# Bioinfo-Tools/PANGEA-plus

Hardware: AMD Instinct MI355X
Metric: classified reads/sec (+ HBM GB/s fraction), 150 bp vs 1 Gbp db, 1/2/4/8 GPU (higher is better)
Workload: dtype u64 (2-bit packed bases, integer scores)

## Files before the change

include/pangea_hip.h:

```cpp
#ifndef PANGEA_HIP_H
#define PANGEA_HIP_H

#include <stddef.h>
#include <stdint.h>

#ifdef __cplusplus
extern "C" {
#endif

typedef enum {
	PGX_OK = 0,
	PGX_E_ARG = -1,
	PGX_E_IO = -2,
	PGX_E_NODEVICE = -3,
	PGX_E_FORMAT = -4,
	PGX_E_NOMEM = -5,
	PGX_E_REFHANG = -6,
	PGX_E_LIMIT = -7
} pgx_status;

const char *pgx_last_error(void);
const char *pgx_version(void);
int pgx_init(int device);
int pgx_device_count(void);
// ... 18 lines not shown
	int64_t n_seq, n_bases;
	int32_t has_amb, index_bits;
	int64_t n_postings;
	int32_t synthetic_ids;
} pgx_db_shape;
int pgx_db_get_shape(const pgx_db *db, pgx_db_shape *out);
int pgx_db_alloc_like(const pgx_db_shape *shape, pgx_db **out);
int pgx_db_finish_import(pgx_db *db);
int pgx_db_checksum(pgx_db *db, uint64_t out[4]);

typedef struct {
	const char *query_path;
	const char *db_prefix;
	const char *out_path;
	int outfmt;
	int rank, world_size;
	int ungapped;
	int no_dust;
} pgx_blastn_opts;
int pgx_blastn_run(const pgx_blastn_opts *opts);
int pgx_db_set_ungapped(pgx_db *db, int ungapped);
int pgx_db_set_dust(pgx_db *db, int dust);
int pgx_db_set_dust_each_search(pgx_db *db, int on);

typedef struct {
	const char *reads_path;
	const char *db_prefix;
	const char *out_path;
	const char *unmapped_path;
	int match_mode;
	int repeat_mode;
	int max_n;
	int report_id;
	const char *reads_b_path;
	const char *unpaired_path;
	int min_insert, max_insert;
} pgx_soap_opts;
int pgx_soap_index(const char *fasta_path);
int pgx_soap_run(const pgx_soap_opts *opts);
int pgx_soap_run_seeded(const pgx_soap_opts *opts, int seed_len, int max_total_mis);

typedef struct pgx_taxdb pgx_taxdb;
typedef struct {
	int32_t tax_id, parent_tax_id;
	int8_t rank;
	char embl_code[3];
// ... 34 lines not shown
	int64_t n_seq;
	int32_t seq_len;
	int64_t n_genus;
	uint64_t read_seed;
	int32_t read_len;
} pgx_synth_cfg;
void pgx_synth_default(pgx_synth_cfg *cfg);
int pgx_db_from_synth(const pgx_synth_cfg *cfg, pgx_db **out);
int pgx_synth_write_taxdump(const pgx_synth_cfg *cfg, const char *dir);

typedef struct pgx_reads pgx_reads;
int pgx_reads_from_fasta(const char *path, int64_t first, int64_t count, pgx_reads **out);
int pgx_reads_from_fasta_text(const char *text, size_t len, int64_t first, int64_t count, pgx_reads **out);
int pgx_reads_from_synth(const pgx_synth_cfg *cfg, int64_t first, int64_t count, pgx_reads **out);
int pgx_reads_write_fasta(const pgx_reads *r, const char *path);
int pgx_reads_redo_dust(pgx_reads *r);
void pgx_reads_close(pgx_reads *r);
int64_t pgx_reads_count(const pgx_reads *r);
int pgx_reads_get(const pgx_reads *r, int64_t i, uint8_t *bases_out, int32_t cap, int32_t *len_out);
int pgx_reads_get_dust(const pgx_reads *r, uint8_t *any_out, uint32_t *woff_out, uint64_t *mask_out, uint64_t *win_f_out,
		       uint64_t *win_r_out, int64_t cap_words, int64_t *n_words_out);
int pgx_db_get_dust(pgx_db *db, const pgx_reads *r, uint8_t *any_out, uint32_t *woff_out, uint64_t *mask_out, uint64_t *win_f_out,
		    uint64_t *win_r_out, int64_t cap_words, int64_t *n_words_out);

typedef struct {
	int32_t read, subject;
	int32_t qstart, qend;
	int32_t sstart, send;
	int32_t score;
	uint16_t mismatch;
	uint16_t gapopen;
} pgx_hit;
#define PGX_HIT_QSPAN(h) ((h).qend - (h).qstart + 1)
#define PGX_HIT_SSPAN(h) (((h).send > (h).sstart ? (h).send - (h).sstart : (h).sstart - (h).send) + 1)
#define PGX_HIT_DIFFS(h) ((PGX_HIT_QSPAN(h) + PGX_HIT_SSPAN(h) - 2 * (h).score - ((PGX_HIT_QSPAN(h) + PGX_HIT_SSPAN(h)) & 1)) / 6)
#define PGX_HIT_GAPS(h) (PGX_HIT_DIFFS(h) - (int32_t)(h).mismatch)
#define PGX_HIT_LENGTH(h) ((PGX_HIT_QSPAN(h) + PGX_HIT_SSPAN(h) + PGX_HIT_GAPS(h)) / 2)

typedef struct pgx_hits pgx_hits;
int pgx_blast_search(pgx_db *db, pgx_reads *reads, pgx_hits **out);
void pgx_hits_close(pgx_hits *h);
int64_t pgx_hits_count(const pgx_hits *h);
int pgx_hits_copy(const pgx_hits *h, pgx_hit *out, int64_t cap);
int pgx_hits_read_offsets(const pgx_hits *h, int64_t *out, int64_t cap);
int pgx_hits_read_counts(const pgx_hits *h, int64_t *out, int64_t cap);
int pgx_hits_slice(const pgx_hits *h, int64_t first_read, int64_t n_reads, pgx_hits **out);
// ... 88 lines not shown
```

pangea-plus_amd/_capi.py:

```python
import ctypes as C
import os
import sys
import threading

import numpy as np

_HERE = os.path.dirname(os.path.abspath(__file__))
lib_path = os.path.join(_HERE, "lib", "libpangea_hip.so")


class PangeaError(RuntimeError):
    def __init__(self, status, msg):
        super().__init__("pangea_hip status %d: %s" % (status, msg))
        self.status = status


_lib = None


def lib():
    global _lib
    if _lib is None:
        if not os.path.exists(lib_path):
            raise PangeaError(-3, "libpangea_hip.so is not built (run `python pangea-plus_amd/build.py`); "
# ... 38 lines not shown
                ("n_postings", C.c_int64), ("synthetic_ids", C.c_int32)]


class _BlastnOpts(C.Structure):
    _fields_ = [("query_path", C.c_char_p), ("db_prefix", C.c_char_p), ("out_path", C.c_char_p), ("outfmt", C.c_int),
                ("rank", C.c_int), ("world_size", C.c_int), ("ungapped", C.c_int), ("no_dust", C.c_int)]


class _SoapOpts(C.Structure):
    _fields_ = [("reads_path", C.c_char_p), ("db_prefix", C.c_char_p), ("out_path", C.c_char_p),
                ("unmapped_path", C.c_char_p), ("match_mode", C.c_int), ("repeat_mode", C.c_int), ("max_n", C.c_int),
                ("report_id", C.c_int), ("reads_b_path", C.c_char_p), ("unpaired_path", C.c_char_p), ("min_insert", C.c_int),
                ("max_insert", C.c_int)]


HIT_DTYPE = np.dtype([("read", "<i4"), ("subject", "<i4"), ("qstart", "<i4"), ("qend", "<i4"), ("sstart", "<i4"),
                      ("send", "<i4"), ("score", "<i4"), ("mismatch", "<u2"), ("gapopen", "<u2")])
REC_DTYPE = np.dtype([("hit", "<i4"), ("matches", "<i4")])
VOTE_DTYPE = np.dtype([("depth", "<i4"), ("name", "<u4", (7,)), ("votes", "u1", (7,)), ("pad", "u1")])

SYMBOLS = [
    "pgx_last_error", "pgx_version", "pgx_init", "pgx_device_count", "pgx_current_device", "pgx_db_build", "pgx_db_open",
    "pgx_db_from_fasta", "pgx_db_close", "pgx_db_num_seqs", "pgx_db_num_bases", "pgx_db_seq_id",
    "pgx_db_device_arrays", "pgx_db_get_shape", "pgx_db_alloc_like", "pgx_db_finish_import", "pgx_db_checksum", "pgx_blastn_run", "pgx_db_set_ungapped", "pgx_db_set_dust", "pgx_db_set_dust_each_search",
    "pgx_soap_index", "pgx_soap_run", "pgx_soap_run_seeded", "pgx_tax_create", "pgx_tax_open", "pgx_tax_close", "pgx_tax_gi2taxid",
    "pgx_tax_node", "pgx_tax_names", "pgx_tax_format_node", "pgx_tax_format_name", "pgx_tax_cli", "pgx_free",
    "pgx_tax_lineage_batch", "pgx_taxcollect_file", "pgx_consensus_file", "pgx_synth_default", "pgx_db_from_synth",
    "pgx_synth_write_taxdump", "pgx_reads_from_fasta", "pgx_reads_from_fasta_text", "pgx_reads_from_synth", "pgx_reads_write_fasta", "pgx_reads_redo_dust", "pgx_rdp_write_file", "pgx_reads_close", "pgx_reads_count",
    "pgx_reads_get", "pgx_reads_get_dust", "pgx_db_get_dust", "pgx_blast_search", "pgx_hits_close", "pgx_hits_count", "pgx_hits_copy",
    "pgx_hits_read_offsets", "pgx_hits_read_counts", "pgx_hits_slice", "pgx_hits_format", "pgx_db_bind_taxonomy", "pgx_db_subject_lineage",
    "pgx_rdp_from_file", "pgx_rdp_from_synth", "pgx_rdp_close", "pgx_consensus_batch", "pgx_classify_consensus", "pgx_classify_consensus_tri", "pgx_vote3_batch", "pgx_vote3_format",
    "pgx_consensus_format", "pgx_consensus_format_file", "pgx_last_stage_times", "pgx_megaclust_file", "pgx_megaclust_batch", "pgx_megaclustable", "pgx_unclas_file", "pgx_unclassified_batch", "pgx_trim_file", "pgx_trim_reads", "pgx_blast_score_columns", "pgx_blast_score_columns_v", "pgx_probe_gather", "pgx_probe_issue", "pgx_probe_issue_name",
]


def _declare(L):
    def sig(name, restype=C.c_int, argtypes=None):
        f = getattr(L, name, None)
        if f is None:
            return
        f.restype = restype
        if argtypes is not None:
            f.argtypes = argtypes
    V, I64, I32, S = C.c_void_p, C.c_int64, C.c_int32, C.c_char_p
    sig("pgx_last_error", S)
    sig("pgx_version", S)
    sig("pgx_db_num_seqs", I64, [V])
    sig("pgx_db_num_bases", I64, [V])
    sig("pgx_db_seq_id", S, [V, I64])
    sig("pgx_db_subject_lineage", S, [V, I64])
    sig("pgx_db_set_ungapped", C.c_int, [V, C.c_int])
    sig("pgx_db_set_dust_each_search", C.c_int, [V, C.c_int])
    sig("pgx_reads_count", I64, [V])
    sig("pgx_hits_count", I64, [V])
    sig("pgx_reads_from_synth", C.c_int, [V, I64, I64, V])
    sig("pgx_reads_from_fasta", C.c_int, [S, I64, I64, V])
    sig("pgx_reads_from_fasta_text", C.c_int, [C.c_char_p, C.c_size_t, I64, I64, V])
    sig("pgx_reads_get", C.c_int, [V, I64, V, I32, V])
    sig("pgx_reads_get_dust", C.c_int, [V, V, V, V, V, V, I64, V])
    sig("pgx_db_get_dust", C.c_int, [V, V, V, V, V, V, V, I64, V])
    sig("pgx_reads_write_fasta", C.c_int, [V, S])
    sig("pgx_reads_redo_dust", C.c_int, [V])
    sig("pgx_rdp_write_file", C.c_int, [V, V, V, S])
    sig("pgx_hits_copy", C.c_int, [V, V, I64])
    sig("pgx_hits_read_offsets", C.c_int, [V, V, I64])
    sig("pgx_hits_read_counts", C.c_int, [V, V, I64])
    sig("pgx_rdp_from_synth", C.c_int, [V, I64, I64, V, V])
    sig("pgx_consensus_batch", C.c_int, [V, V, V, V, I64])
    sig("pgx_classify_consensus", C.c_int, [V, V, V, V, V, I64])
    sig("pgx_classify_consensus_tri", C.c_int, [V, V, V, C.c_char_p, V, V, I64])
    sig("pgx_vote3_batch", C.c_int, [V, V, V, V, C.c_char_p, V, I64])
    sig("pgx_vote3_format", C.c_int, [V, V, V, I64, V, V])
    sig("pgx_consensus_format", C.c_int, [V, V, V, V, I64, V, V])
    sig("pgx_consensus_format_file", C.c_int, [V, V, V, V, I64, S, V])
    sig("pgx_tax_lineage_batch", C.c_int, [V, V, I64, V, V, V])
# ... 123 lines not shown
        s = _DbShape()
        _check(lib().pgx_db_get_shape(self.ptr, C.byref(s)))
        return (s.n_seq, s.n_bases, s.has_amb, s.index_bits, s.n_postings, s.synthetic_ids)

    def checksum(self):
        out = (C.c_uint64 * 4)()
        _check(lib().pgx_db_checksum(self.ptr, out))
        return tuple(int(x) for x in out)

    def device_arrays(self):
        arr = (_DevArray * 16)()
        n = _check(lib().pgx_db_device_arrays(self.ptr, arr, 16))
        return [(arr[i].name.decode(), _CudaArray(arr[i].ptr, arr[i].bytes, self)) for i in range(n)]

    def set_ungapped(self, flag=True):
        _check(lib().pgx_db_set_ungapped(self.ptr, 1 if flag else 0))

    def set_dust(self, flag=True):
        _check(lib().pgx_db_set_dust(self.ptr, 1 if flag else 0))

    def set_dust_each_search(self, flag):
        _check(lib().pgx_db_set_dust_each_search(self.ptr, 1 if flag else 0))

    def dust_bits(self, reads):
        return _dust_bits(lambda *a: lib().pgx_db_get_dust(self.ptr, reads.ptr, *a), len(reads))

    def bind_taxonomy(self, tax):
        _check(lib().pgx_db_bind_taxonomy(self.ptr, tax.ptr))

    def subject_lineage(self, i):
        s = lib().pgx_db_subject_lineage(self.ptr, i)
        return None if s is None else s.decode("latin-1")


def _dust_bits(call, n):
    n_words = C.c_int64()
    _check(call(None, None, None, None, None, 0, C.byref(n_words)))
    nw = n_words.value
    any_ = np.zeros(n, dtype=np.uint8)
    woff = np.zeros(n + 1, dtype=np.uint32)
    mask, win_f, win_r = (np.zeros(max(nw, 1), dtype=np.uint64) for _ in range(3))
    _check(call(any_.ctypes.data, woff.ctypes.data, mask.ctypes.data, win_f.ctypes.data, win_r.ctypes.data, nw, None))
    return any_, woff, mask[:nw], win_f[:nw], win_r[:nw]


class Reads(_Handle):
# ... 342 lines not shown
```

pangea-plus_amd/csrc/classify.hip:

```cpp
#include <algorithm>
#include <chrono>

#include "bitops.hpp"
#include "consensus_core.hpp"
#include "engine.hpp"

namespace pgx {

struct Diag {
	const uint64_t *rw, *ra;
	const uint64_t *dbw, *dba;
	int64_t dstart;
	int lo, hi;
};

template <bool AMB> __device__ __forceinline__ uint64_t mmw(const Diag &D, int w)
{
	int b0 = 32 * w;
	if (b0 + 32 <= D.lo || b0 >= D.hi)
		return kEven;
	uint64_t x = D.rw[w] ^ window64(D.dbw, D.dstart + b0);
	uint64_t m = (x | (x >> 1)) & kEven;
	if (AMB) {
		if (D.ra)
			m |= D.ra[w];
		if (D.dba)
			m |= window64(D.dba, D.dstart + b0);
	}
// ... 229 lines not shown
				return lo - 1;
			w--;
			m = mmw<AMB>(D, w);
		}
		int r = 32 * w + ((63 - __clzll((long long)m)) >> 1);
		return r >= lo ? r : lo - 1;
	}
	struct Fwd {
		int k;
	};
	__device__ __forceinline__ Fwd fwd_from(int k) const { return Fwd{ k }; }
	__device__ __forceinline__ int fwd_next(Fwd &c) const { return c.k = first_ge(c.k + 1); }
	struct Bwd {
		int k;
	};
	__device__ __forceinline__ Bwd bwd_from(int k) const { return Bwd{ k }; }
	__device__ __forceinline__ int bwd_next(Bwd &c) const { return c.k = last_lt(c.k); }
};

constexpr int kStage = 128;
constexpr int kDeal = 2;
constexpr int kQueue = 64 * (kDeal + 1);
constexpr int kWavesPerBlock = 4;

typedef uint32_t u32x4 __attribute__((ext_vector_type(4)));
union HitWords {
	pgx_hit h;
	u32x4 v[2];
};
__device__ __forceinline__ void store_hit_stream(pgx_hit *p, const pgx_hit &h)
{
	HitWords w;
	w.h = h;
	u32x4 *d = reinterpret_cast<u32x4 *>(p);
	__builtin_nontemporal_store(w.v[0], d);
	__builtin_nontemporal_store(w.v[1], d + 1);
}


constexpr int kDiagSlots = 128;
constexpr int kDiagProbes = 8;
constexpr uint32_t kNoDiag = 0xFFFFFFFFu;

struct WaveLds {
	union {
		pgx_hit hit[kStage];
// ... 280 lines not shown
					}
				}
				h.qstart = (int32_t)woff;
				h.qend = anchor;
				h.sstart = (int32_t)(uint32_t)(D.dstart + anchor);
				h.send = strand | (b0l << 1) | (b0r << 12);
				h.score = L;
				h.mismatch = (uint16_t)kl;
				h.gapopen = (uint16_t)kr;
			}
			if (PGX_DBG_STOP(db) != 7)
				emit(h);
			covered = br + 1;
		}
		if constexpr (Mask::kHasWindows) {
			pos = Mask::win_first_ge(W, covered > e ? covered : e + 1);
			if (uw && pos < D.hi)
				pos = M.last_lt(pos) + 1;
		} else
			pos = covered > e + 1 ? covered : e + 1;
	}
}

__device__ __forceinline__ void lds_fence()
{
	asm volatile("s_waitcnt lgkmcnt(0)" ::: "memory");
	__builtin_amdgcn_wave_barrier();
}

template <bool AMB, int NW, bool LISTED, bool DUST>
__global__ __launch_bounds__(64 * kWavesPerBlock, NW == 8 ? 3 : 4) void k_seed_extend(DbView db, ReadsView rd, OutView ov,
								      uint32_t *__restrict__ read_cnt,
								      uint32_t *__restrict__ read_start)
{
	constexpr bool DENSE = NW > 0;
	constexpr int RPW = DENSE ? 2 : 1;
	constexpr int LPR = 64 / RPW;
	constexpr unsigned int SLOT_CAP = kStage;
	__shared__ WaveLds s_lds[kWavesPerBlock];
	const int wave = threadIdx.x >> 6, lane = threadIdx.x & 63;
	const int my_rs = lane / LPR, my_li = lane % LPR;
	WaveLds *st = &s_lds[wave];
	unsigned long long n_probe = 0, n_post = 0, n_runs = 0, n_main = 0, n_surv = 0;
	unsigned long long chunk_base = 0;
	unsigned int chunk_used = kChunk;
	const unsigned long long lt_mask = lane ? (~0ull >> (64 - lane)) : 0ull;

	for (uint32_t rbase = (blockIdx.x * kWavesPerBlock + wave) * RPW; rbase < rd.n; rbase += gridDim.x * kWavesPerBlock * RPW) {
		const bool hasB = RPW == 2 && rbase + 1 < rd.n;
		const uint32_t rA = LISTED ? rd.list[rbase] : rbase, rB = LISTED ? (hasB ? rd.list[rbase + 1] : 0u) : rbase + 1;
		const int LA = (int)rd.len[rA], LB = hasB ? (int)rd.len[rB] : 0;
		const uint32_t wA = rd.woff[rA], wB = hasB ? rd.woff[rB] : 0u;
		const int L = my_rs ? LB : LA;
		const uint32_t w0 = my_rs ? wB : wA;
		const int nps = L >= kSeedK ? (L - kSeedK) / kProbeStride + 1 : 0;
		const int P = 2 * nps;
		const int PA = LA >= kSeedK ? 2 * ((LA - kSeedK) / kProbeStride + 1) : 0;
		const int PB = LB >= kSeedK ? 2 * ((LB - kSeedK) / kProbeStride + 1) : 0;
		const int Pmax = PA > PB ? PA : PB;
		unsigned int emitted[2] = { 0, 0 }, q_n = 0;
		bool frag[2] = { false, false };
		if (lane == 0) {
			st->n[0] = st->n[1] = 0;
			st->direct[0] = st->direct[1] = 0;
		}
		if (RPW == 2) {
#pragma unroll
			for (int k = 0; k < 2 * kDiagSlots / 64; k++)
				(&st->diag[0][0][0])[k * 64 + lane] = kNoDiag;
		}
		const bool dustA = DUST && rd.dustwin_f && rd.dust_any[rA] != 0, dustB = DUST && rd.dustwin_f && hasB && rd.dust_any[rB] != 0;
// ... 959 lines not shown
	v.n_bases = db->n_bases;
	v.bits = db->index_bits;
	v.gapped = db->ungapped ? 0 : 1;
	v.deep_from = kGapDeepFrom;
#ifdef PGX_STAGE_PROBES
	v.dbg_stop = getenv("PGX_SEED_STOP") ? atoi(getenv("PGX_SEED_STOP")) : 0;
#else
	v.dbg_stop = 0;
#endif
	return v;
}

static ReadsView reads_view(const pgx_reads *rd)
{
	ReadsView v;
	v.fwd = rd->d_fwd.data();
	v.rc = rd->d_rc.data();
	v.fwd_amb = rd->has_amb ? rd->d_fwd_amb.data() : nullptr;
	v.rc_amb = rd->has_amb ? rd->d_rc_amb.data() : nullptr;
	v.len = rd->d_len.data();
	v.woff = rd->d_woff.data();
	v.n = (uint32_t)rd->n;
	v.list = nullptr;
	v.dustwin_f = rd->has_dust ? rd->dustb.win_f.data() : nullptr;
	v.dustwin_r = rd->has_dust ? rd->dustb.win_r.data() : nullptr;
	v.dust_any = rd->has_dust ? rd->dustb.any.data() : nullptr;
	return v;
}

static ConsView cons_view(const pgx_db *db, const pgx_rdp *rdp)
{
	ConsView cv;
	memset(&cv, 0, sizeof cv);
#ifdef PGX_STAGE_PROBES
	cv.dbg = getenv("PGX_SORT_STOP") ? atoi(getenv("PGX_SORT_STOP")) : 0;
#else
	cv.dbg = 0;
#endif
	if (db && db->bound) {
		cv.subj_tok_off = db->d_subj_tok_off.data();
		cv.subj_tok = db->d_subj_tok.data();
		cv.tok_rank = db->d_tok_rank.data();
		cv.subj_pairs = db->d_subj_pairs.data();
		cv.pair_words = db->pair_words;
		cv.simrank_lut = db->d_simrank_lut.data();
		cv.simrank_len = db->d_simrank_len.data();
		cv.simrank_undef = db->simrank_undef;
		cv.simrank_zero = db->simrank_zero;
	}
	cv.np_max = db ? db->max_pairs : 15;
	cv.nr_max = rdp ? rdp->max_trip : kRdpRegs;
	if (rdp) {
		cv.rdp_off = rdp->d_off.data();
		cv.rdp_name = rdp->d_name.data();
		cv.rdp_rank = rdp->d_rank.data();
		cv.rdp_present = rdp->d_present.data();
		cv.rdp_code = rdp->d_code.data();
	}
	return cv;
}

struct StageEvents {
	static constexpr int kN = 8;
	hipEvent_t e[kN] = {};
	bool ok = false;
	int init()
	{
		if (ok)
			return 0;
		for (auto &x : e)
			PGX_HIP(hipEventCreate(&x));
		ok = true;
		return 0;
	}
	void mark(int i, hipStream_t s) { (void)hipEventRecord(e[i], s); }
	float ms(int a, int b) const
	{
		float t = 0;
		(void)hipEventElapsedTime(&t, e[a], e[b]);
		return t;
	}
};

__global__ __launch_bounds__(256) void k_merge_pieces(const pgx_hit *__restrict__ scratch, const uint32_t *__restrict__ piece_start,
						      const uint32_t *__restrict__ piece_off, const uint32_t *__restrict__ parent,
						      const uint32_t *__restrict__ qoff, uint32_t n_pieces, pgx_hit *__restrict__ hits,
// ... 26 lines not shown
	if (r > n_reads)
		return;
	const uint32_t o = piece_off[piece_first[r]];
	read_off[r] = o;
	if (r < n_reads) {
		read_cnt[r] = piece_off[piece_first[r + 1]] - o;
		read_start[r] = kFragmented;
	}
}

struct Workspace {
	hipStream_t stream = nullptr;
	StageEvents ev;
	DevBuf<unsigned long long> counters;
	unsigned long long *h_counters = nullptr;
	DevBuf<pgx_hit> scratch, ovf;
	DevBuf<uint8_t> scratch_key, ovf_key;
	DevBuf<uint8_t> scratch_reg;
	DevBuf<uint32_t> partial, cursor, big_list, read_start, mid_list;
	DevBuf<uint32_t> piece_cnt, piece_off, parent_start;
	DevBuf<pgx_consensus_rec> recs;
	GappedWork gapped;
	DustBufs dust;
	pgx_hits hits;
	uint64_t hit_cap_hint = 0, ovf_cap_hint = 0;
	double table_per_read_hint = 0.0;
	pgx_stage_times times;
	int device = -1;
	~Workspace()
	{
		if (h_counters)
			(void)hipHostFree(h_counters);
		if (stream)
			(void)hipStreamDestroy(stream);
	}
};
constexpr int kNCounters = 12;

static int workspace_of(pgx_db *db, Workspace **out)
{
	if (!db->work) {
		auto w = std::make_shared<Workspace>();
		PGX_HIP(hipGetDevice(&w->device));
		PGX_HIP(hipStreamCreate(&w->stream));
		PGX_HIP(hipHostMalloc((void **)&w->h_counters, (kNCounters + 3) * sizeof(unsigned long long)));
		PGX_TRY(w->ev.init());
		PGX_TRY(w->counters.alloc(kNCounters, 0, 0, true));
		db->work = w;
	}
	*out = static_cast<Workspace *>(db->work.get());
	return 0;
}

int db_stream(pgx_db *db, hipStream_t *out)
{
	Workspace *ws = nullptr;
	PGX_TRY(workspace_of(db, &ws));
	*out = ws->stream;
	return 0;
}

int search_pipeline(pgx_db *db, pgx_reads *rd, const pgx_rdp *rdp, pgx_hits *out, pgx_consensus_rec *d_recs)
{
	PGX_TRY(require_device());
	if (rdp && !db->bound)
		return fail(PGX_E_ARG, "consensus needs pgx_db_bind_taxonomy() first");
	if (rdp && rdp->n != rd->n)
		return fail(PGX_E_ARG, "RDP stream holds %lld reads, batch holds %lld", (long long)rdp->n, (long long)rd->n);
	std::lock_guard<std::mutex> lock(db->search_mu);
	static const bool laps_on = getenv("PGX_CALL_LAPS") != nullptr;
	const auto lap_t0 = std::chrono::steady_clock::now();
	auto lap = [&](const char *what) {
		if (laps_on)
			fprintf(stderr, "[pgx lap] %8.2f ms  %s\n", std::chrono::duration<double, std::milli>(std::chrono::steady_clock::now() - lap_t0).count(), what);
	};
	trace_point("search_pipeline: entered");
	Workspace *wsp = nullptr;
	PGX_TRY(workspace_of(db, &wsp));
	Workspace &ws = *wsp;
	hipStream_t st = ws.stream;
	pgx_stage_times &tm = ws.times;
	memset(&tm, 0, sizeof tm);
	const uint64_t n = (uint64_t)rd->n;
	out->n_reads = rd->n;
	PGX_TRY(out->d_read_cnt.ensure(n + 1));
	PGX_TRY(out->d_read_off.ensure(n + 1));
	if (n == 0) {
		out->n_hits = 0;
		t_times = tm;
		return 0;
	}
	index_check(db, "search_pipeline");
	const DbView dv = db_view(db);
	const bool split = rd->pieces && rd->pieces->n > 0;
	const pgx_reads *sr = split ? rd->pieces.get() : rd;
	const uint64_t ns = (uint64_t)sr->n;
	if (split) {
		PGX_TRY(ws.piece_cnt.ensure(ns + 1));
		PGX_TRY(ws.piece_off.ensure(ns + 1));
		PGX_TRY(ws.parent_start.ensure(n));
	}
	ReadsView rv = reads_view(sr);
	if (!db->dust)
		rv.dustwin_f = rv.dustwin_r = nullptr;
	const int grid = (int)std::min<uint64_t>((n + kWavesPerBlock - 1) / kWavesPerBlock, 256ull * 8);
// ... 9 lines not shown
	bool long_reads = false;
	for (auto &c : classes)
		long_reads = long_reads || c.words == 0;
	const uint32_t n_part = (uint32_t)((ns + kScanBlock * kScanItems - 1) / (kScanBlock * kScanItems));
	PGX_TRY(ws.partial.ensure(n_part));
	PGX_TRY(ws.cursor.ensure(ns));
	PGX_TRY(ws.big_list.ensure(n));
	PGX_TRY(ws.mid_list.ensure(n + 64ull * kWavesPerBlock * 256 * 8));
	trace_point("search_pipeline: lists ready");
	const ConsView cv = cons_view(db, rdp);
	const int lds_ok = rd->max_len <= 65535 ? 1 : 0;
	uint64_t H = 0, H_ovf = 0;
	ws.ev.mark(6, st);
	const bool dust_now = db->dust && db->dust_each_search;
	if (dust_now) {
		PGX_TRY(reads_dust_again(sr, ws.dust, st));
		if (sr->has_dust) {
			rv.dustwin_f = ws.dust.win_f.data();
			rv.dustwin_r = ws.dust.win_r.data();
			rv.dust_any = ws.dust.any.data();
		}
	}
	ws.ev.mark(7, st);
	for (int attempt = 0;; attempt++) {
		if (attempt > 8)
			return fail(PGX_E_LIMIT, "hit tables did not settle after %d attempts", attempt);
		PGX_TRY(scratch.ensure(cap));
		PGX_TRY(ovf.ensure(ovf_cap));
		trace_point("search_pipeline: seed tables ready");
		PGX_TRY(out->d_hits.ensure(table_cap));
		trace_point("search_pipeline: hit table ready");
		cap = scratch.n;
		ovf_cap = ovf.n;
		if (dv.gapped) {
			PGX_TRY(ws.scratch_key.ensure(cap + 16));
			PGX_TRY(ws.scratch_reg.ensure(cap + 16));
			PGX_TRY(ws.ovf_key.ensure(ovf_cap));
			PGX_HIP(hipMemsetAsync(ws.scratch_key.data(), 0xFF, cap + 16, st));
		}
		table_cap = out->d_hits.n;
		PGX_HIP(hipMemsetAsync(ws.counters.data(), 0, kNCounters * sizeof(unsigned long long), st));
		OutView ov;
		ov.main = scratch.data();
		ov.ovf = ovf.data();
		ov.main_key = ws.scratch_key.data();
		ov.ovf_key = ws.ovf_key.data();
		ov.main_reg = ws.scratch_reg.data();
		ov.reg_shift = gapped_region_shift(db->n_bases);
		ov.main_cap = cap;
		ov.ovf_cap = ovf_cap;
		ov.counters = ws.counters.data();
		uint32_t *big_count = reinterpret_cast<uint32_t *>(ws.counters.data() + 8), *mid_count = reinterpret_cast<uint32_t *>(ws.counters.data() + 9);
		trace_point("search_pipeline: tables ready");
		lap("tables ready");
		ws.ev.mark(0, st);
		uint32_t *rc_ptr = split ? ws.piece_cnt.data() : out->d_read_cnt.data(), *rs_ptr = read_start.data();
		for (const pgx_reads::SearchClass &c0 : classes) {
			pgx_reads::SearchClass c = c0;
			c.amb = c.amb || db->has_amb;
			ReadsView cvw = rv;
			const uint64_t cn = c.count;
			cvw.n = (uint32_t)cn;
			cvw.list = c.listed ? sr->d_class_list.data() + c.off : nullptr;
			const int per_block = kWavesPerBlock * (c.words > 0 ? 2 : 1);
			const dim3 g((unsigned)std::min<uint64_t>((cn + per_block - 1) / per_block, 256ull * 8)), b(64 * kWavesPerBlock);
#define PGX_SEED_LAUNCH2(A, W, D)                                                                                                  \
	do {                                                                                                                       \
		if (c.listed)                                                                                                      \
			hipLaunchKernelGGL((k_seed_extend<A, W, true, D>), g, b, 0, st, dv, cvw, ov, rc_ptr, rs_ptr);             \
		else                                                                                                               \
			hipLaunchKernelGGL((k_seed_extend<A, W, false, D>), g, b, 0, st, dv, cvw, ov, rc_ptr, rs_ptr);            \
	} while (0)
#define PGX_SEED_LAUNCH(A, W)                                                                                                      \
	do {                                                                                                                       \
		if (c.dust && cvw.dustwin_f)                                                                                       \
			PGX_SEED_LAUNCH2(A, W, true);                                                                              \
		else                                                                                                               \
			PGX_SEED_LAUNCH2(A, W, false);                                                                             \
	} while (0)
			if (c.amb && c.words == 3)
				PGX_SEED_LAUNCH(true, 3);
			else if (c.amb && c.words == 5)
				PGX_SEED_LAUNCH(true, 5);
			else if (c.amb && c.words == 8)
				PGX_SEED_LAUNCH(true, 8);
			else if (c.amb)
// ... 86 lines not shown
			again = true;
			tm.grown |= 4;
		}
		if (!again && H > table_cap) {
			table_cap = H + H / 16;
			again = true;
			tm.grown |= 8;
		}
		tm.attempts = attempt + 1;
		if (!again)
			break;
	}
	ws.hit_cap_hint = std::max<uint64_t>(ws.hit_cap_hint, h_cnt[0] + h_cnt[0] / 16);
	ws.ovf_cap_hint = std::max<uint64_t>(ws.ovf_cap_hint, H_ovf + H_ovf / 16);
	ws.table_per_read_hint = std::max(ws.table_per_read_hint, (double)(H + H / 16) / (double)std::max(n, ns));
	out->n_hits = (int64_t)H;
	out->gapped = dv.gapped != 0;
	tm.hits = (int64_t)H;
	tm.probes = (int64_t)h_cnt[1];
	tm.postings = (int64_t)h_cnt[2];
	tm.candidates = (int64_t)h_cnt[3];
	tm.survivors = (int64_t)h_cnt[6];
	tm.gapped_wide = (int64_t)(uint32_t)h_cnt[kNCounters] + (int64_t)(uint32_t)(h_cnt[kNCounters + 2] >> 32);
	tm.seed_extend_ms = ws.ev.ms(0, 1);
	tm.gapped_ms = ws.ev.ms(1, 2);
	tm.group_ms = ws.ev.ms(2, 3);
	tm.sort_ms = ws.ev.ms(3, 4);
	tm.total_ms = ws.ev.ms(0, 4);
	tm.dust_ms = dust_now ? ws.ev.ms(6, 7) : 0.0f;
	tm.total_ms += tm.dust_ms;
	const unsigned long long hit_limit = getenv("PGX_HIT_LIMIT") ? strtoull(getenv("PGX_HIT_LIMIT"), nullptr, 10) : (1ull << 32);
	if (H >= hit_limit)
		return fail(PGX_E_LIMIT, "%llu hits in one batch exceed the 32-bit slot limit: use smaller batches",
			    (unsigned long long)H);
	const uint32_t n_big = (uint32_t)h_cnt[8];
	if (n_big) {
		const uint32_t *sort_start = split ? ws.parent_start.data() : read_start.data();
		ws.ev.mark(4, st);
		PGX_TRY(sort_big_reads(out->d_hits.data(), scratch.data(), sort_start, out->d_read_off.data(), out->d_read_cnt.data(),
				       ws.big_list.data(), n_big, dv.gapped != 0));
		if (rdp) {
			hipLaunchKernelGGL(k_consensus_serial, dim3((n_big + 63) / 64), dim3(64), 0, 0, out->d_hits.data(), out->d_read_off.data(),
					   out->d_read_cnt.data(), ws.big_list.data(), n_big, cv, d_recs);
			PGX_HIP(hipGetLastError());
		}
		ws.ev.mark(5, 0);
		PGX_HIP(hipDeviceSynchronize());
		const float extra = ws.ev.ms(4, 5);
		tm.sort_ms += extra;
		tm.total_ms += extra;
	}
// ... 71 lines not shown
	}
	return pgx_classify_consensus(db, reads, rdp, hits_out, out, cap);
}

int pgx_db_get_dust(pgx_db *db, const pgx_reads *r, uint8_t *any_out, uint32_t *woff_out, uint64_t *mask_out, uint64_t *win_f_out,
		    uint64_t *win_r_out, int64_t cap_words, int64_t *n_words_out)
{
	if (!db || !r)
		return fail(PGX_E_ARG, "pgx_db_get_dust: null argument");
	if (r->pieces && r->pieces->n > 0)
		return fail(PGX_E_ARG, "pgx_db_get_dust: the batch is searched piece by piece, the handle's bits describe the pieces");
	std::lock_guard<std::mutex> lock(db->search_mu);
	if (!db->work)
		return fail(PGX_E_ARG, "pgx_db_get_dust: no search has run through this handle");
	const Workspace &ws = *static_cast<const Workspace *>(db->work.get());
	return dust_read_back("pgx_db_get_dust", r, ws.dust, ws.stream, any_out, woff_out, mask_out, win_f_out, win_r_out, cap_words, n_words_out);
}

int pgx_db_set_dust_each_search(pgx_db *db, int on)
{
	if (!db)
		return fail(PGX_E_ARG, "pgx_db_set_dust_each_search: null argument");
	db->dust_each_search = on != 0;
	return 0;
}

int pgx_db_set_ungapped(pgx_db *db, int ungapped)
{
	if (!db)
		return fail(PGX_E_ARG, "pgx_db_set_ungapped: null argument");
	std::lock_guard<std::mutex> lock(db->search_mu);
	db->ungapped = ungapped != 0;
	return 0;
}

int pgx_db_set_dust(pgx_db *db, int dust)
{
	if (!db)
		return fail(PGX_E_ARG, "pgx_db_set_dust: null argument");
	std::lock_guard<std::mutex> lock(db->search_mu);
	db->dust = dust != 0;
	return 0;
}

void pgx_hits_close(pgx_hits *h) { delete h; }
int64_t pgx_hits_count(const pgx_hits *h) { return h ? h->n_hits : 0; }
// ... 69 lines not shown
```

pangea-plus_amd/csrc/engine.hpp:

```cpp
#pragma once
#include <memory>
#include <functional>
#include <thread>
#include <atomic>
#include <mutex>
#include <string>
#include <unordered_map>
#include <vector>

#include "common.hpp"
#include "rdp_host.hpp"

struct pgx_db {
	int64_t n_seq = 0, n_bases = 0;
	bool has_amb = false;
	bool synthetic_ids = false;
	std::vector<uint32_t> h_seq_off;
	std::vector<std::string> ids;
	std::vector<uint64_t> h_words, h_amb;

	pgx::DevBuf<uint64_t> d_words, d_amb;
	pgx::DevBuf<uint32_t> d_seq_off, d_blk_subj;
	pgx::DevBuf<uint4> d_blk_info;
	pgx::DevBuf<uint32_t> d_amb_blk;
	int index_bits = 0;
	int64_t n_postings = 0;
	std::shared_ptr<void> work;
	std::mutex search_mu;
	bool dust = true;
	bool dust_each_search = false;
	bool ungapped = false;
	pgx::DevBuf<uint32_t> d_bucket_off, d_postings;
	pgx::DevBuf<uint3> d_post_ctx;

	bool bound = false;
	std::vector<std::string> lineage;
	std::vector<std::string> token_text;
	std::unordered_map<std::string, uint32_t> token_id;
	pgx::DevBuf<uint32_t> d_subj_tok_off, d_subj_tok;
	pgx::DevBuf<int8_t> d_tok_rank;
	pgx::DevBuf<uint32_t> d_subj_pairs;
	int max_pairs = 15;
	int pair_words = 16;
	std::vector<int8_t> h_tok_rank;
	std::vector<int32_t> subj_taxid;
	std::vector<std::string> lin_text;
	pgx::DevBuf<uint32_t> d_subj_lin;
	uint32_t empty_lin = 0;
	pgx::DevBuf<uint32_t> d_node_name_tok;
	pgx::DevBuf<uint32_t> d_simrank_lut;
	pgx::DevBuf<uint32_t> d_simrank_len;
	uint32_t simrank_undef = 0, simrank_zero = 0;
	uint32_t intern(const std::string &s);
// ... 165 lines not shown
#endif

struct DbView {
	const uint64_t *words, *amb;
	const uint32_t *seq_off, *blk_subj, *bucket_off, *postings;
	const uint4 *blk_info;
	const uint3 *post_ctx;
	const uint32_t *amb_blk;
	uint32_t n_seq;
	int64_t n_bases;
	int bits;
	int gapped;
	int deep_from;
	int dbg_stop;
};

struct ReadsView {
	const uint64_t *fwd, *rc, *fwd_amb, *rc_amb;
	const uint64_t *dustwin_f, *dustwin_r;
	const uint8_t *dust_any;
	const uint32_t *len, *woff;
	uint32_t n;
	const uint32_t *list;
};


constexpr uint32_t kFragmented = 0xFFFFFFFFu;

struct GappedWork {
	DevBuf<unsigned long long> big_list, big_list2;
	DevBuf<uint32_t> big_count;
	DevBuf<uint2> side_list;
	DevBuf<uint32_t> order;
	DevBuf<uint32_t> items, bins;
	DevBuf<uint32_t> items1;
	DevBuf<uint8_t> keys1;
};
int gapped_stage(const DbView &dv, const ReadsView &rv, pgx_hit *main_table, const uint8_t *main_key, const uint32_t *read_start,
		 const uint32_t *read_cnt, pgx_hit *ovf_table, const uint8_t *ovf_key, const unsigned long long *ovf_count, unsigned long long ovf_cap, bool long_reads,
		 unsigned long long hit_cap, int max_len, GappedWork &gw, hipStream_t stream, const unsigned long long *main_used, const uint8_t *main_reg);
constexpr int kGapDeepFrom = 320;
inline int gapped_region_shift(int64_t n_bases)
{
	int s = 0;
	while (((n_bases + 1024) >> s) > 240)
		s++;
// ... 22 lines not shown
```

Baseline: 136.0 million.

## Sort reads by probable database locus before seeding and hand them out by ticket

Adds a pre-pass that looks up one or two 16-mers of each read in the seed index, takes the first posting's database position as a coarse bin, and radix-sorts reads by that bin. The seed/extend kernel then walks the sorted list, pulling work from an atomic ticket counter instead of a static stride. The aim is that waves running at the same time touch nearby database regions, which should improve cache reuse of the reference words and posting lists, and that dynamic ticketing should balance load. This costs an extra key kernel, a rocprim sort, some buffers and an atomic per grab. It only switches on automatically for large batches against large databases.

```diff
diff --git a/include/pangea_hip.h b/include/pangea_hip.h
--- a/include/pangea_hip.h
+++ b/include/pangea_hip.h
@@ -64,6 +64,7 @@
 int pgx_db_set_ungapped(pgx_db *db, int ungapped);
 int pgx_db_set_dust(pgx_db *db, int dust);
 int pgx_db_set_dust_each_search(pgx_db *db, int on);
+int pgx_db_set_read_order(pgx_db *db, int mode);
 
 typedef struct {
 	const char *reads_path;
@@ -144,6 +145,7 @@
 		       uint64_t *win_r_out, int64_t cap_words, int64_t *n_words_out);
 int pgx_db_get_dust(pgx_db *db, const pgx_reads *r, uint8_t *any_out, uint32_t *woff_out, uint64_t *mask_out, uint64_t *win_f_out,
 		    uint64_t *win_r_out, int64_t cap_words, int64_t *n_words_out);
+int pgx_db_get_read_order(pgx_db *db, const pgx_reads *r, uint32_t *order_out, uint32_t *key_out, int64_t cap, int64_t *n_out);
 
 typedef struct {
 	int32_t read, subject;
diff --git a/pangea-plus_amd/_capi.py b/pangea-plus_amd/_capi.py
--- a/pangea-plus_amd/_capi.py
+++ b/pangea-plus_amd/_capi.py
@@ -84,7 +84,7 @@
 SYMBOLS = [
     "pgx_last_error", "pgx_version", "pgx_init", "pgx_device_count", "pgx_current_device", "pgx_db_build", "pgx_db_open",
     "pgx_db_from_fasta", "pgx_db_close", "pgx_db_num_seqs", "pgx_db_num_bases", "pgx_db_seq_id",
-    "pgx_db_device_arrays", "pgx_db_get_shape", "pgx_db_alloc_like", "pgx_db_finish_import", "pgx_db_checksum", "pgx_blastn_run", "pgx_db_set_ungapped", "pgx_db_set_dust", "pgx_db_set_dust_each_search",
+    "pgx_db_device_arrays", "pgx_db_get_shape", "pgx_db_alloc_like", "pgx_db_finish_import", "pgx_db_checksum", "pgx_blastn_run", "pgx_db_set_ungapped", "pgx_db_set_dust", "pgx_db_set_dust_each_search", "pgx_db_set_read_order", "pgx_db_get_read_order",
     "pgx_soap_index", "pgx_soap_run", "pgx_soap_run_seeded", "pgx_tax_create", "pgx_tax_open", "pgx_tax_close", "pgx_tax_gi2taxid",
     "pgx_tax_node", "pgx_tax_names", "pgx_tax_format_node", "pgx_tax_format_name", "pgx_tax_cli", "pgx_free",
     "pgx_tax_lineage_batch", "pgx_taxcollect_file", "pgx_consensus_file", "pgx_synth_default", "pgx_db_from_synth",
@@ -113,6 +113,8 @@
     sig("pgx_db_subject_lineage", S, [V, I64])
     sig("pgx_db_set_ungapped", C.c_int, [V, C.c_int])
     sig("pgx_db_set_dust_each_search", C.c_int, [V, C.c_int])
+    sig("pgx_db_set_read_order", C.c_int, [V, C.c_int])
+    sig("pgx_db_get_read_order", C.c_int, [V, V, V, V, I64, V])
     sig("pgx_reads_count", I64, [V])
     sig("pgx_hits_count", I64, [V])
     sig("pgx_reads_from_synth", C.c_int, [V, I64, I64, V])
@@ -282,6 +284,17 @@
     def set_dust_each_search(self, flag):
         _check(lib().pgx_db_set_dust_each_search(self.ptr, 1 if flag else 0))
 
+    def set_read_order(self, mode):
+        _check(lib().pgx_db_set_read_order(self.ptr, int(mode)))
+
+    def read_order(self, reads):
+        n = C.c_int64()
+        _check(lib().pgx_db_get_read_order(self.ptr, reads.ptr, None, None, 0, C.byref(n)))
+        order, keys = np.zeros(n.value, dtype=np.uint32), np.zeros(n.value, dtype=np.uint32)
+        if n.value:
+            _check(lib().pgx_db_get_read_order(self.ptr, reads.ptr, order.ctypes.data, keys.ctypes.data, n.value, C.byref(n)))
+        return order, keys
+
     def dust_bits(self, reads):
         return _dust_bits(lambda *a: lib().pgx_db_get_dust(self.ptr, reads.ptr, *a), len(reads))
 
diff --git a/pangea-plus_amd/csrc/classify.hip b/pangea-plus_amd/csrc/classify.hip
--- a/pangea-plus_amd/csrc/classify.hip
+++ b/pangea-plus_amd/csrc/classify.hip
@@ -4,6 +4,9 @@
 #include "bitops.hpp"
 #include "consensus_core.hpp"
 #include "engine.hpp"
+#include "read_order.hpp"
+
+#include <rocprim/device/device_radix_sort.hpp>
 
 namespace pgx {
 
@@ -279,6 +282,7 @@
 constexpr int kDeal = 2;
 constexpr int kQueue = 64 * (kDeal + 1);
 constexpr int kWavesPerBlock = 4;
+constexpr int kOrderGrab = 4;
 
 typedef uint32_t u32x4 __attribute__((ext_vector_type(4)));
 union HitWords {
@@ -605,6 +609,49 @@
 	}
 }
 
+struct OrderIndexView {
+	const uint32_t *bucket_off, *postings;
+	int bits;
+	__device__ __forceinline__ OrderRange range(uint32_t kmer) const
+	{
+		const uint32_t b = seed_bucket(kmer, bits);
+		const uint32_t lo = __builtin_nontemporal_load(&bucket_off[b]);
+		return OrderRange{ lo, __builtin_nontemporal_load(&bucket_off[(uint64_t)b + 1]) - lo };
+	}
+	__device__ __forceinline__ uint32_t first(uint32_t lo) const { return __builtin_nontemporal_load(&postings[lo]); }
+};
+
+__global__ __launch_bounds__(256) void k_read_order_keys(DbView db, ReadsView rd, int shift, uint32_t last_bin, uint32_t cls,
+							 uint32_t *__restrict__ keys, uint32_t *__restrict__ vals)
+{
+	const uint32_t i = blockIdx.x * blockDim.x + threadIdx.x;
+	if (i >= rd.n)
+		return;
+	const uint32_t r = rd.list ? rd.list[i] : i;
+	const int L = (int)rd.len[r];
+	uint32_t kmer[2][2] = { { 0, 0 }, { 0, 0 } };
+	bool usable[2][2] = { { false, false }, { false, false } };
+	if (L >= kOrderProbeLen) {
+		const uint32_t w0 = rd.woff[r];
+		const bool two = L >= kOrderProbe1 + kOrderProbeLen;
+#pragma unroll
+		for (int s = 0; s < 2; s++) {
+			const uint64_t *rw = (s ? rd.rc : rd.fwd) + w0;
+			const uint64_t *ra = s ? rd.rc_amb : rd.fwd_amb;
+			const uint64_t a = ra ? ra[w0] : 0ull;
+			kmer[s][0] = window16(rw, kOrderProbe0);
+			usable[s][0] = (uint32_t)a == 0u;
+			if (two) {
+				kmer[s][1] = window16(rw, kOrderProbe1);
+				usable[s][1] = (uint32_t)(a >> (2 * kOrderProbe1)) == 0u;
+			}
+		}
+	}
+	const OrderIndexView ix = { db.bucket_off, db.postings, db.bits };
+	keys[i] = read_order_key(ix, kmer, usable, shift, last_bin) | (cls << 16);
+	vals[i] = r;
+}
+
 __device__ __forceinline__ void lds_fence()
 {
 	asm volatile("s_waitcnt lgkmcnt(0)" ::: "memory");
@@ -629,7 +676,22 @@
 	unsigned int chunk_used = kChunk;
 	const unsigned long long lt_mask = lane ? (~0ull >> (64 - lane)) : 0ull;
 
-	for (uint32_t rbase = (blockIdx.x * kWavesPerBlock + wave) * RPW; rbase < rd.n; rbase += gridDim.x * kWavesPerBlock * RPW) {
+	uint32_t t_next = 0, t_end = 0;
+	auto next_round = [&](uint32_t cur) -> uint32_t {
+		if (!LISTED || !rd.ticket)
+			return cur + gridDim.x * kWavesPerBlock * RPW;
+		if (t_next == t_end) {
+			uint32_t t = 0;
+			if (lane == 0)
+				t = atomicAdd(rd.ticket, (uint32_t)(kOrderGrab * RPW));
+			t_next = __builtin_amdgcn_readfirstlane(t);
+			t_end = t_next + kOrderGrab * RPW;
+		}
+		const uint32_t r = t_next;
+		t_next += RPW;
+		return r;
+	};
+	for (uint32_t rbase = LISTED && rd.ticket ? next_round(0) : (blockIdx.x * kWavesPerBlock + wave) * RPW; rbase < rd.n; rbase = next_round(rbase)) {
 		const bool hasB = RPW == 2 && rbase + 1 < rd.n;
 		const uint32_t rA = LISTED ? rd.list[rbase] : rbase, rB = LISTED ? (hasB ? rd.list[rbase + 1] : 0u) : rbase + 1;
 		const int LA = (int)rd.len[rA], LB = hasB ? (int)rd.len[rB] : 0;
@@ -1635,6 +1697,7 @@
 	v.woff = rd->d_woff.data();
 	v.n = (uint32_t)rd->n;
 	v.list = nullptr;
+	v.ticket = nullptr;
 	v.dustwin_f = rd->has_dust ? rd->dustb.win_f.data() : nullptr;
 	v.dustwin_r = rd->has_dust ? rd->dustb.win_r.data() : nullptr;
 	v.dust_any = rd->has_dust ? rd->dustb.any.data() : nullptr;
@@ -1674,7 +1737,7 @@
 }
 
 struct StageEvents {
-	static constexpr int kN = 8;
+	static constexpr int kN = 10;
 	hipEvent_t e[kN] = {};
 	bool ok = false;
 	int init()
@@ -1747,6 +1810,10 @@
 	DevBuf<pgx_consensus_rec> recs;
 	GappedWork gapped;
 	DustBufs dust;
+	DevBuf<uint32_t> order_key_in, order_val_in, order_key, order_list;
+	DevBuf<uint8_t> order_tmp;
+	DevBuf<uint32_t> order_ticket;
+	uint64_t order_n = 0;
 	pgx_hits hits;
 	uint64_t hit_cap_hint = 0, ovf_cap_hint = 0;
 	double table_per_read_hint = 0.0;
@@ -1782,6 +1849,63 @@
 	Workspace *ws = nullptr;
 	PGX_TRY(workspace_of(db, &ws));
 	*out = ws->stream;
+	return 0;
+}
+
+constexpr uint64_t kOrderMinReads = 1u << 22;
+constexpr uint64_t kOrderMinDbBytes = 32ull << 20;
+static bool order_wanted(const pgx_db *db, uint64_t class_reads)
+{
+	if (db->read_order == 1)
+		return class_reads > 0;
+	if (db->read_order == 2)
+		return false;
+	return class_reads >= kOrderMinReads && (uint64_t)db->n_bases / 4 >= kOrderMinDbBytes;
+}
+
+static int order_reads(const pgx_db *db, const DbView &dv, const ReadsView &rv, const pgx_reads *sr, Workspace &ws,
+		       std::vector<int64_t> &ordered)
+{
+	hipStream_t st = ws.stream;
+	const std::vector<pgx_reads::SearchClass> &classes = sr->classes;
+	ordered.assign(classes.size(), -1);
+	const int shift = read_order_shift(dv.n_bases), key_bits = read_order_key_bits(dv.n_bases);
+	const uint32_t last_bin = read_order_last_bin(dv.n_bases);
+	uint64_t total = 0;
+	size_t tmp_bytes = 0;
+	for (size_t c = 0; c < classes.size(); c++)
+		if (order_wanted(db, classes[c].count)) {
+			ordered[c] = (int64_t)total;
+			total += classes[c].count;
+			size_t bytes = 0;
+			PGX_HIP(rocprim::radix_sort_pairs(nullptr, bytes, (uint32_t *)nullptr, (uint32_t *)nullptr, (uint32_t *)nullptr, (uint32_t *)nullptr,
+							  (size_t)classes[c].count, 0, key_bits, st));
+			tmp_bytes = std::max(tmp_bytes, bytes);
+		}
+	ws.order_n = total;
+	if (total == 0)
+		return 0;
+	PGX_TRY(ws.order_key_in.ensure(total));
+	PGX_TRY(ws.order_val_in.ensure(total));
+	PGX_TRY(ws.order_key.ensure(total));
+	PGX_TRY(ws.order_list.ensure(total));
+	PGX_TRY(ws.order_tmp.ensure(tmp_bytes ? tmp_bytes : 1));
+	PGX_TRY(ws.order_ticket.ensure(classes.size()));
+	for (size_t c = 0; c < classes.size(); c++) {
+		if (ordered[c] < 0)
+			continue;
+		const uint64_t o = (uint64_t)ordered[c], cn = classes[c].count;
+		ReadsView cvw = rv;
+		cvw.n = (uint32_t)cn;
+		cvw.list = classes[c].listed ? sr->d_class_list.data() + classes[c].off : nullptr;
+		hipLaunchKernelGGL(k_read_order_keys, dim3((unsigned)((cn + 255) / 256)), dim3(256), 0, st, dv, cvw, shift, last_bin, (uint32_t)c,
+				   ws.order_key_in.data() + o, ws.order_val_in.data() + o);
+		PGX_HIP(hipGetLastError());
+		size_t bytes = ws.order_tmp.n;
+		PGX_HIP(rocprim::radix_sort_pairs(ws.order_tmp.data(), bytes, ws.order_key_in.data() + o, ws.order_key.data() + o,
+						  ws.order_val_in.data() + o, ws.order_list.data() + o, (size_t)cn, 0, key_bits, st));
+	}
+	trace_point("order_reads");
 	return 0;
 }
 
@@ -1806,6 +1930,7 @@
 	hipStream_t st = ws.stream;
 	pgx_stage_times &tm = ws.times;
 	memset(&tm, 0, sizeof tm);
+	ws.order_n = 0;
 	const uint64_t n = (uint64_t)rd->n;
 	out->n_reads = rd->n;
 	PGX_TRY(out->d_read_cnt.ensure(n + 1));
@@ -1861,6 +1986,11 @@
 		}
 	}
 	ws.ev.mark(7, st);
+	std::vector<int64_t> ordered;
+	PGX_TRY(order_reads(db, dv, rv, sr, ws, ordered));
+	const bool order_now = ws.order_n > 0;
+	if (order_now)
+		ws.ev.mark(8, st);
 	for (int attempt = 0;; attempt++) {
 		if (attempt > 8)
 			return fail(PGX_E_LIMIT, "hit tables did not settle after %d attempts", attempt);
@@ -1892,15 +2022,22 @@
 		uint32_t *big_count = reinterpret_cast<uint32_t *>(ws.counters.data() + 8), *mid_count = reinterpret_cast<uint32_t *>(ws.counters.data() + 9);
 		trace_point("search_pipeline: tables ready");
 		lap("tables ready");
+		if (order_now)
+			PGX_HIP(hipMemsetAsync(ws.order_ticket.data(), 0, classes.size() * sizeof(uint32_t), st));
 		ws.ev.mark(0, st);
 		uint32_t *rc_ptr = split ? ws.piece_cnt.data() : out->d_read_cnt.data(), *rs_ptr = read_start.data();
-		for (const pgx_reads::SearchClass &c0 : classes) {
-			pgx_reads::SearchClass c = c0;
+		for (size_t ci = 0; ci < classes.size(); ci++) {
+			pgx_reads::SearchClass c = classes[ci];
 			c.amb = c.amb || db->has_amb;
 			ReadsView cvw = rv;
 			const uint64_t cn = c.count;
 			cvw.n = (uint32_t)cn;
 			cvw.list = c.listed ? sr->d_class_list.data() + c.off : nullptr;
+			if (ordered[ci] >= 0) {
+				c.listed = true;
+				cvw.list = ws.order_list.data() + ordered[ci];
+				cvw.ticket = ws.order_ticket.data() + ci;
+			}
 			const int per_block = kWavesPerBlock * (c.words > 0 ? 2 : 1);
 			const dim3 g((unsigned)std::min<uint64_t>((cn + per_block - 1) / per_block, 256ull * 8)), b(64 * kWavesPerBlock);
 #define PGX_SEED_LAUNCH2(A, W, D)                                                                                                  \
@@ -2033,11 +2170,11 @@
 	tm.candidates = (int64_t)h_cnt[3];
 	tm.survivors = (int64_t)h_cnt[6];
 	tm.gapped_wide = (int64_t)(uint32_t)h_cnt[kNCounters] + (int64_t)(uint32_t)(h_cnt[kNCounters + 2] >> 32);
-	tm.seed_extend_ms = ws.ev.ms(0, 1);
+	tm.seed_extend_ms = ws.ev.ms(0, 1) + (order_now ? ws.ev.ms(7, 8) : 0.0f);
 	tm.gapped_ms = ws.ev.ms(1, 2);
 	tm.group_ms = ws.ev.ms(2, 3);
 	tm.sort_ms = ws.ev.ms(3, 4);
-	tm.total_ms = ws.ev.ms(0, 4);
+	tm.total_ms = ws.ev.ms(0, 4) + (order_now ? ws.ev.ms(7, 8) : 0.0f);
 	tm.dust_ms = dust_now ? ws.ev.ms(6, 7) : 0.0f;
 	tm.total_ms += tm.dust_ms;
 	const unsigned long long hit_limit = getenv("PGX_HIT_LIMIT") ? strtoull(getenv("PGX_HIT_LIMIT"), nullptr, 10) : (1ull << 32);
@@ -2155,6 +2292,39 @@
 	if (!db)
 		return fail(PGX_E_ARG, "pgx_db_set_dust_each_search: null argument");
 	db->dust_each_search = on != 0;
+	return 0;
+}
+
+int pgx_db_set_read_order(pgx_db *db, int mode)
+{
+	if (!db || mode < 0 || mode > 2)
+		return fail(PGX_E_ARG, "pgx_db_set_read_order: null handle, or a mode other than 0 (auto), 1 (always), 2 (never)");
+	std::lock_guard<std::mutex> lock(db->search_mu);
+	db->read_order = mode;
+	return 0;
+}
+
+int pgx_db_get_read_order(pgx_db *db, const pgx_reads *r, uint32_t *order_out, uint32_t *key_out, int64_t cap, int64_t *n_out)
+{
+	if (!db || !r || !n_out)
+		return fail(PGX_E_ARG, "pgx_db_get_read_order: null argument");
+	std::lock_guard<std::mutex> lock(db->search_mu);
+	if (!db->work)
+		return fail(PGX_E_ARG, "pgx_db_get_read_order: no search has run through this handle");
+	const Workspace &ws = *static_cast<const Workspace *>(db->work.get());
+	const pgx_reads *sr = r->pieces && r->pieces->n > 0 ? r->pieces.get() : r;
+	if ((int64_t)ws.order_n > sr->n)
+		return fail(PGX_E_ARG, "pgx_db_get_read_order: the last search through this handle was given another batch");
+	*n_out = (int64_t)ws.order_n;
+	if (!order_out && !key_out)
+		return 0;
+	if (cap < (int64_t)ws.order_n)
+		return fail(PGX_E_ARG, "pgx_db_get_read_order: room for %lld entries, the list holds %lld", (long long)cap, (long long)ws.order_n);
+	PGX_HIP(hipStreamSynchronize(ws.stream));
+	if (order_out)
+		PGX_TRY(ws.order_list.download(order_out, (size_t)ws.order_n));
+	if (key_out)
+		PGX_TRY(ws.order_key.download(key_out, (size_t)ws.order_n));
 	return 0;
 }
 
diff --git a/pangea-plus_amd/csrc/engine.hpp b/pangea-plus_amd/csrc/engine.hpp
--- a/pangea-plus_amd/csrc/engine.hpp
+++ b/pangea-plus_amd/csrc/engine.hpp
@@ -29,6 +29,7 @@
 	std::mutex search_mu;
 	bool dust = true;
 	bool dust_each_search = false;
+	int read_order = 0;
 	bool ungapped = false;
 	pgx::DevBuf<uint32_t> d_bucket_off, d_postings;
 	pgx::DevBuf<uint3> d_post_ctx;
@@ -240,6 +241,7 @@
 	const uint32_t *len, *woff;
 	uint32_t n;
 	const uint32_t *list;
+	uint32_t *ticket;
 };
 
 
diff --git a/pangea-plus_amd/csrc/read_order.hpp b/pangea-plus_amd/csrc/read_order.hpp
--- /dev/null
+++ b/pangea-plus_amd/csrc/read_order.hpp
@@ -0,0 +1,64 @@
+#pragma once
+#include <cstdint>
+
+#if defined(__HIPCC__)
+#define PGX_HD __host__ __device__
+#else
+#define PGX_HD
+#endif
+
+namespace pgx {
+
+constexpr int kOrderProbe0 = 0, kOrderProbe1 = 13;
+constexpr int kOrderProbeLen = 16;
+constexpr uint32_t kOrderMaxBins = 65536;
+
+PGX_HD inline int read_order_shift(int64_t n_bases)
+{
+	const int64_t top = n_bases > 0 ? n_bases - 1 : 0;
+	int s = 0;
+	while ((top >> s) + 2 > (int64_t)kOrderMaxBins)
+		s++;
+	return s;
+}
+PGX_HD inline uint32_t read_order_last_bin(int64_t n_bases)
+{
+	const int64_t top = n_bases > 0 ? n_bases - 1 : 0;
+	return (uint32_t)(top >> read_order_shift(n_bases)) + 1u;
+}
+PGX_HD inline int read_order_key_bits(int64_t n_bases)
+{
+	const uint32_t last = read_order_last_bin(n_bases);
+	int b = 1;
+	while (b < 32 && (last >> b) != 0)
+		b++;
+	return b;
+}
+
+struct OrderRange {
+	uint32_t lo, cnt;
+};
+
+template <class Index>
+PGX_HD inline uint32_t read_order_key(const Index &ix, const uint32_t kmer[2][2], const bool usable[2][2], int shift, uint32_t last_bin)
+{
+	const OrderRange none = { 0u, 0u };
+	const OrderRange f0 = usable[0][0] ? ix.range(kmer[0][0]) : none, r0 = usable[1][0] ? ix.range(kmer[1][0]) : none;
+	uint32_t lo;
+	if (f0.cnt != r0.cnt)
+		lo = r0.cnt > f0.cnt ? r0.lo : f0.lo;
+	else {
+		const OrderRange f1 = usable[0][1] ? ix.range(kmer[0][1]) : none, r1 = usable[1][1] ? ix.range(kmer[1][1]) : none;
+		const bool rev = r1.cnt > f1.cnt;
+		if (f0.cnt)
+			lo = rev ? r0.lo : f0.lo;
+		else if (f1.cnt | r1.cnt)
+			lo = rev ? r1.lo : f1.lo;
+		else
+			return last_bin;
+	}
+	const uint32_t bin = ix.first(lo) >> shift;
+	return bin < last_bin ? bin : last_bin;
+}
+
+}
```

Result: faster. 139.1 million, median of 6 (+2.3%).
